# aspuru-guzik-group/waveflow

Measured on AMD Instinct MI355X. Metric: flow log-prob evals/sec, higher is better.
Workload: dtype f32

## Files before the change

### waveflow_amd/csrc/wf_kernels_scalar.hip

```cpp
#include "wf_scalar_impl.h"

namespace wf {

namespace scalar {
WF_SCALAR_SHAPE(extern, 2, 32) WF_SCALAR_SHAPE(extern, 3, 32) WF_SCALAR_SHAPE(extern, 4, 32) WF_SCALAR_SHAPE(extern, 5, 32)
WF_SCALAR_SHAPE(extern, 6, 32) WF_SCALAR_SHAPE(extern, 7, 32) WF_SCALAR_SHAPE(extern, 8, 32)
WF_SCALAR_SHAPE(extern, 2, 64) WF_SCALAR_SHAPE(extern, 3, 64) WF_SCALAR_SHAPE(extern, 4, 64) WF_SCALAR_SHAPE(extern, 5, 64)
WF_SCALAR_SHAPE(extern, 6, 64) WF_SCALAR_SHAPE(extern, 7, 64) WF_SCALAR_SHAPE(extern, 8, 64)
}

namespace {
using namespace scalar;

constexpr int kSumBlock = 256;
constexpr int kSumMaxBlocks = 1024;

__device__ __forceinline__ void block_reduce2(double& a, double& b, double* sm) {
    sm[threadIdx.x] = a;
    sm[kSumBlock + threadIdx.x] = b;
    __syncthreads();
    for (int s = kSumBlock / 2; s > 0; s >>= 1) {
        if ((int)threadIdx.x < s) {
            sm[threadIdx.x] += sm[threadIdx.x + s];
            sm[kSumBlock + threadIdx.x] += sm[kSumBlock + threadIdx.x + s];
        }
        __syncthreads();
    }
    a = sm[0];
    b = sm[kSumBlock];
}

__device__ __forceinline__ void ring_push(double s, double q, double n, double* __restrict__ ring, int ring_len, unsigned long long* __restrict__ counter) {
    const unsigned long long c = *counter;
    double* slot = ring + (c % (unsigned long long)ring_len) * 3;
    slot[0] = s; slot[1] = q; slot[2] = n;
    *counter = c + 1;
}

__global__ __launch_bounds__(kSumBlock) void k_sums_stage1(const float* __restrict__ v, int64_t B, double* __restrict__ partial,
                                                           double* __restrict__ final, double* __restrict__ ring, int ring_len,
                                                           unsigned long long* __restrict__ counter) {
    __shared__ double sm[2 * kSumBlock];
    double s = 0.0, q = 0.0;
    for (int64_t i = (int64_t)blockIdx.x * kSumBlock + threadIdx.x; i < B; i += (int64_t)gridDim.x * kSumBlock) {
        const double x = (double)v[i];
        s += x;
        q += x * x;
    }
    block_reduce2(s, q, sm);
    if (threadIdx.x == 0) {
        if (final) {
            final[0] = s;
            final[1] = q;
            final[2] = (double)B;
            if (ring) ring_push(s, q, (double)B, ring, ring_len, counter);
        } else {
            partial[2 * blockIdx.x] = s;
            partial[2 * blockIdx.x + 1] = q;
        }
    }
}

__global__ __launch_bounds__(kSumBlock) void k_sums_stage2(const double* __restrict__ partial, int n_blocks, int64_t B, double* __restrict__ out,
                                                           double* __restrict__ ring, int ring_len, unsigned long long* __restrict__ counter) {
    __shared__ double sm[2 * kSumBlock];
    double s = 0.0, q = 0.0;
    for (int i = threadIdx.x; i < n_blocks; i += kSumBlock) {
        s += partial[2 * i];
        q += partial[2 * i + 1];
    }
    block_reduce2(s, q, sm);
    if (threadIdx.x == 0) {
        out[0] = s;
        out[1] = q;
        out[2] = (double)B;
        if (ring) ring_push(s, q, (double)B, ring, ring_len, counter);
    }
}

int sums_blocks(int64_t B) {
    int64_t n = (B + kSumBlock - 1) / kSumBlock;
    if (n < 1) n = 1;
    if (n > kSumMaxBlocks) n = kSumMaxBlocks;
    return (int)n;
}

int finish_launch() {
    hipError_t e = hipGetLastError();
    if (e != hipSuccess) {
        set_hip_error((int)e);
        return WF_ERR_HIP;
    }
    return WF_OK;
}

}

#define WF_DISPATCH_D(D_, NBP_, CALL)                                         \
    if ((NBP_) == 32) {                                                          \
        switch (D_) {                                                            \
            case 2: CALL(2, 32); break;                                          \
            case 3: CALL(3, 32); break;                                          \
            case 4: CALL(4, 32); break;                                          \
            case 5: CALL(5, 32); break;                                          \
            case 6: CALL(6, 32); break;                                          \
            case 7: CALL(7, 32); break;                                          \
            case 8: CALL(8, 32); break;                                          \
            default: return WF_ERR_UNSUPPORTED;                                  \
        }                                                                        \
    } else if ((NBP_) == 64) {                                                   \
        switch (D_) {                                                            \
            case 2: CALL(2, 64); break;                                          \
            case 3: CALL(3, 64); break;                                          \
            case 4: CALL(4, 64); break;                                          \
            case 5: CALL(5, 64); break;                                          \
            case 6: CALL(6, 64); break;                                          \
            case 7: CALL(7, 64); break;                                          \
            case 8: CALL(8, 64); break;                                          \
            default: return WF_ERR_UNSUPPORTED;                                  \
        }                                                                        \
    } else {                                                                     \
        return WF_ERR_UNSUPPORTED;                                               \
    }

int launch_scalar(const ModelDev& md, const ModelDev* md_dev, int mode, const float* x, int64_t B, float* out, float* u, int32_t* idx,
                  void* stream) {
    hipStream_t s = (hipStream_t)stream;
#define CALL(DD, NN) run_eval<DD, NN>(md_dev, mode, x, B, out, u, idx, s)
    WF_DISPATCH_D(md.D, md.nbp, CALL)
#undef CALL
    return finish_launch();
}

int launch_scalar_layer(const ModelDev& md, const ModelDev* md_dev, int layer, const float* u_in, int64_t B, float* y, float* logdet,
                        int32_t* idx, void* stream) {
    hipStream_t s = (hipStream_t)stream;
#define CALL(DD, NN) run_layer<DD, NN>(md_dev, layer, u_in, B, y, logdet, idx, s)
    WF_DISPATCH_D(md.D, md.nbp, CALL)
#undef CALL
    return finish_launch();
}

int launch_scalar_inverse(const ModelDev& md, const ModelDev* md_dev, const float* u, int64_t B, float* x, int exact, void* stream) {
    hipStream_t s = (hipStream_t)stream;
#define CALL(DD, NN) run_inverse<DD, NN>(md_dev, u, B, x, exact, s)
    WF_DISPATCH_D(md.D, md.nbp, CALL)
#undef CALL
    return finish_launch();
}

int launch_scalar_sample(const ModelDev& md, const ModelDev* md_dev, unsigned long long seed, int64_t B, float* x, float* latent, int exact,
                         void* stream) {
    hipStream_t s = (hipStream_t)stream;
#define CALL(DD, NN) run_sample<DD, NN>(md_dev, seed, B, x, latent, exact, s)
    WF_DISPATCH_D(md.D, md.nbp, CALL)
#undef CALL
    return finish_launch();
}

__global__ void k_sort_rows(const float* __restrict__ x, int64_t B, int D, float* __restrict__ xs, int32_t* __restrict__ inv) {
    const int64_t b = (int64_t)blockIdx.x * blockDim.x + threadIdx.x;
    if (b >= B) return;
    float r[WF_MAX_DIM];
    for (int d = 0; d < D; ++d) r[d] = x[b * D + d];
    int n = 0;
    for (int pass = 0; pass < D; ++pass)
        for (int i = pass & 1; i + 1 < D; i += 2)
            if (r[i] > r[i + 1]) {
                const float t = r[i]; r[i] = r[i + 1]; r[i + 1] = t;
                ++n;
            }
    if (xs)
        for (int d = 0; d < D; ++d) xs[b * D + d] = r[d];
    if (inv) inv[b] = n;
}
__global__ void k_apply_sign(float* __restrict__ v, const int32_t* __restrict__ inv, int64_t B) {
    const int64_t b = (int64_t)blockIdx.x * blockDim.x + threadIdx.x;
    if (b < B && (inv[b] & 1)) v[b] = -v[b];
}

int launch_sort_rows(const float* x, int64_t B, int D, float* xs, int32_t* inv, void* stream) {
    if (B <= 0) return WF_OK;
    hipLaunchKernelGGL(k_sort_rows, dim3((unsigned)((B + 255) / 256)), dim3(256), 0, (hipStream_t)stream, x, B, D, xs, inv);
    return finish_launch();
}
int launch_apply_sign(float* v, const int32_t* inv, int64_t B, void* stream) {
    if (B <= 0) return WF_OK;
    hipLaunchKernelGGL(k_apply_sign, dim3((unsigned)((B + 255) / 256)), dim3(256), 0, (hipStream_t)stream, v, inv, B);
    return finish_launch();
}

int64_t block_sums_ws_bytes(int64_t) { return (int64_t)kSumMaxBlocks * 2 * sizeof(double); }

int launch_block_sums(const float* v, int64_t B, double* out, void* ws, int64_t, void* stream, double* ring, int ring_len,
                      unsigned long long* counter) {
    hipStream_t s = (hipStream_t)stream;
    const int nb = sums_blocks(B);
    double* partial = (double*)ws;
    if (nb == 1) {
        hipLaunchKernelGGL(k_sums_stage1, dim3(1), dim3(kSumBlock), 0, s, v, B, partial, out, ring, ring_len, counter);
        return finish_launch();
    }
    hipLaunchKernelGGL(k_sums_stage1, dim3(nb), dim3(kSumBlock), 0, s, v, B, partial, (double*)nullptr, (double*)nullptr, 0,
                       (unsigned long long*)nullptr);
    hipLaunchKernelGGL(k_sums_stage2, dim3(1), dim3(kSumBlock), 0, s, (const double*)partial, nb, B, out, ring, ring_len, counter);
    return finish_launch();
}

}
```

Baseline: 3.861 billion.

## Fuse two-stage block-sum reduction into one kernel via last-block ticket

Replaces the two-launch sum/sum-of-squares reduction with a single kernel. Each block publishes its partials with agent-scope atomics and bumps a per-stream ticket counter, and the last block to finish does the final reduction. Per-stream ticket slots are managed on the host with a mutex and map, and it falls back to the two-stage path when no slot is available. It also unrolls the grid-stride load loop by four. The cost targeted is the extra kernel launch and its dependency, in exchange for fences, atomics and a host-side lookup per call.

Measured after the change: 3.601 billion. 0.933x the previous value.

```diff
diff --git a/waveflow_amd/csrc/wf_kernels_scalar.hip b/waveflow_amd/csrc/wf_kernels_scalar.hip
--- a/waveflow_amd/csrc/wf_kernels_scalar.hip
+++ b/waveflow_amd/csrc/wf_kernels_scalar.hip
@@ -1,3 +1,6 @@
+#include <mutex>
+#include <unordered_map>
+
 #include "wf_scalar_impl.h"
 
 namespace wf {
@@ -37,16 +40,57 @@
     *counter = c + 1;
 }
 
+__device__ __forceinline__ void thread_sums(const float* __restrict__ v, int64_t B, double& s, double& q) {
+    s = 0.0;
+    q = 0.0;
+    const int64_t stride = (int64_t)gridDim.x * kSumBlock;
+    int64_t i = (int64_t)blockIdx.x * kSumBlock + threadIdx.x;
+    for (; i + 3 * stride < B; i += 4 * stride) {
+        float x4[4];
+#pragma unroll
+        for (int u = 0; u < 4; ++u) x4[u] = v[i + u * stride];
+#pragma unroll
+        for (int u = 0; u < 4; ++u) {
+            const double x = (double)x4[u];
+            s += x;
+            q += x * x;
+        }
+    }
+    for (; i < B; i += stride) {
+        const double x = (double)v[i];
+        s += x;
+        q += x * x;
+    }
+}
+
+template <bool kCoherent>
+__device__ __forceinline__ void reduce_partials(const double* partial, int n_blocks, int64_t B, double* __restrict__ out, double* __restrict__ ring,
+                                                int ring_len, unsigned long long* __restrict__ counter, double* sm) {
+    double s = 0.0, q = 0.0;
+    for (int i = threadIdx.x; i < n_blocks; i += kSumBlock) {
+        if (kCoherent) {
+            s += __hip_atomic_load(partial + 2 * i, __ATOMIC_RELAXED, __HIP_MEMORY_SCOPE_AGENT);
+            q += __hip_atomic_load(partial + 2 * i + 1, __ATOMIC_RELAXED, __HIP_MEMORY_SCOPE_AGENT);
+        } else {
+            s += partial[2 * i];
+            q += partial[2 * i + 1];
+        }
+    }
+    block_reduce2(s, q, sm);
+    if (threadIdx.x == 0) {
+        out[0] = s;
+        out[1] = q;
+        out[2] = (double)B;
+        if (ring) ring_push(s, q, (double)B, ring, ring_len, counter);
+    }
+}
+
 __global__ __launch_bounds__(kSumBlock) void k_sums_stage1(const float* __restrict__ v, int64_t B, double* __restrict__ partial,
                                                            double* __restrict__ final, double* __restrict__ ring, int ring_len,
                                                            unsigned long long* __restrict__ counter) {
     __shared__ double sm[2 * kSumBlock];
-    double s = 0.0, q = 0.0;
-    for (int64_t i = (int64_t)blockIdx.x * kSumBlock + threadIdx.x; i < B; i += (int64_t)gridDim.x * kSumBlock) {
-        const double x = (double)v[i];
-        s += x;
-        q += x * x;
-    }
+    double s, q;
+    thread_sums(v, B, s, q);
     block_reduce2(s, q, sm);
     if (threadIdx.x == 0) {
         if (final) {
@@ -64,18 +108,34 @@
 __global__ __launch_bounds__(kSumBlock) void k_sums_stage2(const double* __restrict__ partial, int n_blocks, int64_t B, double* __restrict__ out,
                                                            double* __restrict__ ring, int ring_len, unsigned long long* __restrict__ counter) {
     __shared__ double sm[2 * kSumBlock];
-    double s = 0.0, q = 0.0;
-    for (int i = threadIdx.x; i < n_blocks; i += kSumBlock) {
-        s += partial[2 * i];
-        q += partial[2 * i + 1];
-    }
+    reduce_partials<false>(partial, n_blocks, B, out, ring, ring_len, counter, sm);
+}
+
+constexpr int kSumTickets = 1024;
+__device__ unsigned int g_sums_ticket[kSumTickets];
+
+__global__ __launch_bounds__(kSumBlock) void k_sums_fused(const float* __restrict__ v, int64_t B, double* partial, int slot,
+                                                          double* __restrict__ out, double* __restrict__ ring, int ring_len,
+                                                          unsigned long long* __restrict__ counter) {
+    __shared__ double sm[2 * kSumBlock];
+    __shared__ int is_last;
+    double s, q;
+    thread_sums(v, B, s, q);
     block_reduce2(s, q, sm);
     if (threadIdx.x == 0) {
-        out[0] = s;
-        out[1] = q;
-        out[2] = (double)B;
-        if (ring) ring_push(s, q, (double)B, ring, ring_len, counter);
-    }
+        __hip_atomic_store(partial + 2 * blockIdx.x, s, __ATOMIC_RELAXED, __HIP_MEMORY_SCOPE_AGENT);
+        __hip_atomic_store(partial + 2 * blockIdx.x + 1, q, __ATOMIC_RELAXED, __HIP_MEMORY_SCOPE_AGENT);
+        __builtin_amdgcn_fence(__ATOMIC_RELEASE, "agent");
+        asm volatile("s_waitcnt vmcnt(0)" ::: "memory");
+        const unsigned int t = __hip_atomic_fetch_add(&g_sums_ticket[slot], 1u, __ATOMIC_RELAXED, __HIP_MEMORY_SCOPE_AGENT);
+        __builtin_amdgcn_fence(__ATOMIC_ACQUIRE, "agent");
+        asm volatile("s_waitcnt vmcnt(0)" ::: "memory");
+        is_last = t == gridDim.x - 1;
+    }
+    __syncthreads();
+    if (!is_last) return;
+    reduce_partials<true>(partial, (int)gridDim.x, B, out, ring, ring_len, counter, sm);
+    if (threadIdx.x == 0) __hip_atomic_store(&g_sums_ticket[slot], 0u, __ATOMIC_RELAXED, __HIP_MEMORY_SCOPE_AGENT);
 }
 
 int sums_blocks(int64_t B) {
@@ -192,6 +252,24 @@
 
 int64_t block_sums_ws_bytes(int64_t) { return (int64_t)kSumMaxBlocks * 2 * sizeof(double); }
 
+static int sums_ticket_slot(hipStream_t s) {
+    static std::mutex mu;
+    static std::unordered_map<hipStream_t, int> by_stream;
+    static int next = 0;
+    hipStreamCaptureStatus cap = hipStreamCaptureStatusNone;
+    if (hipStreamIsCapturing(s, &cap) != hipSuccess) {
+        (void)hipGetLastError();
+        return -1;
+    }
+    std::lock_guard<std::mutex> lock(mu);
+    if (cap != hipStreamCaptureStatusNone) return next < kSumTickets ? next++ : -1;
+    auto it = by_stream.find(s);
+    if (it != by_stream.end()) return it->second;
+    if (next >= kSumTickets) return -1;
+    by_stream.emplace(s, next);
+    return next++;
+}
+
 int launch_block_sums(const float* v, int64_t B, double* out, void* ws, int64_t, void* stream, double* ring, int ring_len,
                       unsigned long long* counter) {
     hipStream_t s = (hipStream_t)stream;
@@ -201,6 +279,11 @@
         hipLaunchKernelGGL(k_sums_stage1, dim3(1), dim3(kSumBlock), 0, s, v, B, partial, out, ring, ring_len, counter);
         return finish_launch();
     }
+    const int slot = sums_ticket_slot(s);
+    if (slot >= 0) {
+        hipLaunchKernelGGL(k_sums_fused, dim3(nb), dim3(kSumBlock), 0, s, v, B, partial, slot, out, ring, ring_len, counter);
+        return finish_launch();
+    }
     hipLaunchKernelGGL(k_sums_stage1, dim3(nb), dim3(kSumBlock), 0, s, v, B, partial, (double*)nullptr, (double*)nullptr, 0,
                        (unsigned long long*)nullptr);
     hipLaunchKernelGGL(k_sums_stage2, dim3(1), dim3(kSumBlock), 0, s, (const double*)partial, nb, B, out, ring, ring_len, counter);
```
